# musaru/Fall_Multimodal

Hardware: AMD Instinct MI355X
Metric: clips/sec (fwd+bwd) 3-stream Fall3, B=256, 1/2/4/8 GPUs; top-1 acc parity (higher is better)
Workload: dtype bf16x3; 1 GPU; fall3_3stream_coco_mmpose_V18_S6_B256_per_gpu; global_batch=256, seq_len=30, parallelism=dp1, joints=18, imu_axes=6, classes=11, hip_graph=False, ranks=1

## Files before the change

fall_multimodal_amd/_lib.py:

```python
from __future__ import annotations

import ctypes
import os

import torch

HERE = os.path.dirname(os.path.abspath(__file__))
LIB_PATH = os.environ.get("F3_LIB") or os.path.join(HERE, "libfall3.so")

EXPORTS = (
    "f3_net_create", "f3_net_destroy", "f3_net_num_entries", "f3_net_entry", "f3_net_param_count",
    "f3_net_buffer_count", "f3_net_counter_count", "f3_net_workspace_bytes", "f3_net_forward",
    "f3_net_loss", "f3_net_backward", "f3_rmsprop_step", "f3_conv_forward", "f3_status_string",
    "f3_net_debug_tensor", "f3_conv_backward_data", "f3_conv_backward_weight", "f3_conv_wgrad_packed", "f3_split_x3cat",
    "f3_conv_forward_x3cat", "f3_conv_backward_data_x3cat", "f3_conv_backward_weight_x3cat", "f3_conv_step_x3cat", "f3_graph_mix_forward",
    "f3_graph_mix_backward", "f3_graph_mix_forward_ex", "f3_graph_mix_backward_ex", "f3_net_backward_phase",
    "f3_net_grad_split", "f3_net_wait_phase1", "f3_net_backward_rmsprop", "f3_net_fused_rmsprop", "f3_net_precision", "f3_net_status",
    "f3_targcn_create", "f3_targcn_destroy", "f3_targcn_num_entries", "f3_targcn_entry", "f3_targcn_param_count",
    "f3_targcn_buffer_count", "f3_targcn_workspace_bytes", "f3_targcn_forward", "f3_targcn_backward", "f3_targcn_stage_times", "f3_targcn_status", "f3_net_sensor_times", "f3_soft_ce",
    "f3_sktr_create", "f3_sktr_destroy", "f3_sktr_num_entries", "f3_sktr_entry", "f3_sktr_param_count",
    "f3_sktr_buffer_count", "f3_sktr_counter_count", "f3_sktr_workspace_bytes", "f3_sktr_forward", "f3_sktr_backward",
    "f3_musa_create", "f3_musa_destroy", "f3_musa_num_entries", "f3_musa_entry", "f3_musa_param_count",
    "f3_musa_buffer_count", "f3_musa_counter_count", "f3_musa_workspace_bytes", "f3_musa_forward", "f3_musa_backward",
    "f3_musa_guards",
    "f3_dwconv_t_forward", "f3_pointwise_conv", "f3_rgb_scratch_floats", "f3_rgb_forward", "f3_rgb_backward",
)

F3_OK, F3_EINVAL, F3_EBATCH, F3_EHIP, F3_ESTATE, F3_EDEVICE = 0, 1001, 1002, 1003, 1004, 1005
ENTRY_PARAM, ENTRY_BUFFER, ENTRY_COUNTER = 0, 1, 2


class F3TargcnConfig(ctypes.Structure):
    _fields_ = [(n, ctypes.c_int) for n in ("num_node", "num_class", "precision")]


class F3MusaConfig(ctypes.Structure):
    _fields_ = [(n, ctypes.c_int) for n in ("num_point", "frames", "num_class", "precision")]


class F3SktrConfig(ctypes.Structure):
    _fields_ = [(n, ctypes.c_int) for n in ("num_joint", "frames", "persons", "num_class", "precision")]


class F3Config(ctypes.Structure):
    _fields_ = [(n, ctypes.c_int) for n in (
        "model", "num_node", "num_partition", "num_class", "in_channels", "sensor", "sensor_dim",
        "sensor_classes", "softmax_output", "naming", "frames", "sensor_frames", "precision")]


# ... 14 lines not shown
        "f3_net_num_entries": (I, [P]),
        "f3_net_entry": (I, [P, I, ctypes.POINTER(ctypes.c_char_p), ctypes.POINTER(I), ctypes.POINTER(I),
                             ctypes.POINTER(I64), ctypes.POINTER(I64)]),
        "f3_net_param_count": (I64, [P]),
        "f3_net_buffer_count": (I64, [P]),
        "f3_net_counter_count": (I64, [P]),
        "f3_net_workspace_bytes": (I64, [P, I]),
        "f3_net_forward": (I, [P, I, I, P, P, P, P, P, P, P, P]),
        "f3_net_loss": (I, [P, I, P, P, P, P, P]),
        "f3_net_backward": (I, [P, I, P, P, P, P, P]),
        "f3_net_backward_phase": (I, [P, I, P, P, P, P, I, P]),
        "f3_net_grad_split": (I64, [P]),
        "f3_net_wait_phase1": (I, [P, P]),
        "f3_net_backward_rmsprop": (I, [P, I, P, P, P, P, P, F, F, F, P]),
        "f3_net_fused_rmsprop": (I, [P]),
        "f3_net_precision": (I, [P]),
        "f3_net_status": (I, [P, I]),
        "f3_rmsprop_step": (I, [P, P, P, I64, F, F, F, F, P]),
        "f3_conv_forward": (I, [P, P, P, P, P, I, I, I, I, I, I, I, I, I, P]),
        "f3_status_string": (ctypes.c_char_p, [I]),
        "f3_net_debug_tensor": (P, [P, I, P, I, I, ctypes.c_char_p]),
        "f3_conv_backward_data": (I, [P, P, P, P, I, I, I, I, I, I, I, I, I, P]),
        "f3_conv_backward_weight": (I, [P, P, P, P, I, I, I, I, I, I, I, I, I, P]),
        "f3_conv_wgrad_packed": (I, [P, P, P, ctypes.c_longlong, I, I, I, I, I, I, I, I, P]),
        "f3_split_x3cat": (I, [P, P, ctypes.c_int64, I, P]),
        "f3_conv_forward_x3cat": (I, [P, P, P, P, P, I, I, I, I, I, I, I, I, P]),
        "f3_conv_backward_data_x3cat": (I, [P, P, P, P, I, I, I, I, I, I, I, I, P]),
        "f3_conv_backward_weight_x3cat": (I, [P, P, P, P, I, I, I, I, I, I, I, I, P]),
        "f3_conv_step_x3cat": (I, [I, P, P, P, P, P, P, P, P, P, P, F, P, P, I, I, I, I, I, P]),
        "f3_graph_mix_forward": (I, [P, P, P, I, I, I, I, P]),
        "f3_graph_mix_backward": (I, [P, P, P, P, P, I, I, I, I, P]),
        "f3_graph_mix_forward_ex": (I, [P, P, P, I, I, I, I, I, P]),
        "f3_graph_mix_backward_ex": (I, [P, P, P, P, P, I, I, I, I, I, P]),
        "f3_targcn_create": (I, [ctypes.POINTER(F3TargcnConfig), ctypes.POINTER(P)]),
        "f3_targcn_destroy": (None, [P]),
        "f3_targcn_num_entries": (I, [P]),
        "f3_targcn_entry": (I, [P, I, ctypes.POINTER(ctypes.c_char_p), ctypes.POINTER(I), ctypes.POINTER(I),
                                ctypes.POINTER(I64), ctypes.POINTER(I64)]),
        "f3_targcn_param_count": (I64, [P]),
        "f3_targcn_buffer_count": (I64, [P]),
        "f3_targcn_workspace_bytes": (I64, [P, I]),
        "f3_targcn_stage_times": (I, [P, I, P]),
        "f3_targcn_status": (I, [P, I]),
        "f3_net_sensor_times": (I, [P, I, P]),
        "f3_targcn_forward": (I, [P, I, P, P, P, P, P, P]),
        "f3_targcn_backward": (I, [P, I, P, P, P, P, P, P]),
        "f3_soft_ce": (I, [P, P, I, I, P, P, P]),
        "f3_sktr_create": (I, [ctypes.POINTER(F3SktrConfig), ctypes.POINTER(P)]),
        "f3_sktr_destroy": (None, [P]),
        "f3_sktr_num_entries": (I, [P]),
        "f3_sktr_entry": (I, [P, I, ctypes.POINTER(ctypes.c_char_p), ctypes.POINTER(I), ctypes.POINTER(I),
                              ctypes.POINTER(I64), ctypes.POINTER(I64)]),
        "f3_sktr_param_count": (I64, [P]),
        "f3_sktr_buffer_count": (I64, [P]),
        "f3_sktr_counter_count": (I64, [P]),
        "f3_sktr_workspace_bytes": (I64, [P, I]),
        "f3_sktr_forward": (I, [P, I, I, P, P, P, P, P, P, P, ctypes.c_uint, F, P]),
        "f3_sktr_backward": (I, [P, I, P, P, P, P, P, P]),
        "f3_musa_create": (I, [ctypes.POINTER(F3MusaConfig), ctypes.POINTER(P)]),
        "f3_musa_destroy": (None, [P]),
        "f3_musa_num_entries": (I, [P]),
        "f3_musa_entry": (I, [P, I, ctypes.POINTER(ctypes.c_char_p), ctypes.POINTER(I), ctypes.POINTER(I),
                              ctypes.POINTER(I64), ctypes.POINTER(I64)]),
        "f3_musa_param_count": (I64, [P]),
        "f3_musa_buffer_count": (I64, [P]),
        "f3_musa_counter_count": (I64, [P]),
# ... 39 lines not shown
```

fall_multimodal_amd/csrc/layers.h:

```cpp
#pragma once
#include "common.h"

namespace f3 {

enum : int { PREP_MUL = 0, PREP_PACK_CONV, PREP_PACK_CONV_T, PREP_PACK_GCN, PREP_PACK_GCN_T, PREP_GCN_BIAS, PREP_COPY,
              PREP_UNPACK_CONV };

struct PrepJob {
  int type, n;
  float* dst;
  const float* s0;
  const float* s1;
  const float* s2;
  int d0, d1, d2;
  int bf16;
};

struct DataBnArgs {
  int N, T, V, C, motion;
  const float* skel;
  float* out;
  int act16;
  BnRef bn;
  double* st_sum;
  double* st_sq;
  const float* dout;
  float* dgamma;
  float* dbeta;
  float* part;
};

struct MixArgs {
  int K, V, Cin, frames;
  const float* A;
  const float* x;
  int x16;
  float* z;
  float* dx;
  float* dA;
  int accumulate;
  float* part;
  unsigned short* zb;
  const unsigned short* dzb;
  int no_colsum;
  int x3;
  unsigned short* z3;
};
constexpr int kMixParts = 1024;

struct Gcn0Args {
  int frames, K, V, Ci;
  const float* A;
  const unsigned short* x;
  const unsigned short* w;
  const float* beff;
  unsigned short* z;
  unsigned short* g;
  double* st_sum;
  double* st_sq;
  const unsigned short* dg;
  float* dx;
  int accumulate;
  float* part_dA;
  float* part_dW;
  int f32;
};

struct GcnBiasBwdArgs {
  int K, V, C;
  const float* Aeff;
  const float* A;
  const float* G;
  const float* bias;
  float* db;
  const float* dAeff;
  float* dE;
};

enum : int { RES_NONE = 0, RES_ID = 1, RES_CONV = 2 };

constexpr int kCaMaxRowsPerThread = 4;
// ... 97 lines not shown
  int bchunks;
};


struct BnRunJob {
  const double* sum;
  const double* sumsq;
  double count;
  int C;
  float* rmean;
  float* rvar;
  long long* nbt;
};

constexpr int kMaxPrepJobs = 56;
struct PrepTable {
  int n;
  PrepJob jobs[kMaxPrepJobs];
};
constexpr int kMaxBnJobs = 56;
struct BnRunTable {
  int n;
  BnRunJob jobs[kMaxBnJobs];
};

}

int f3_prep(const f3::PrepTable& t, hipStream_t s);
int f3_databn_fwd(const f3::DataBnArgs* a, hipStream_t s);
int f3_databn_bwd(const f3::DataBnArgs* a, hipStream_t s);
int f3_mix_fwd(const f3::MixArgs* a, hipStream_t s);
int f3_mix_bwd(const f3::MixArgs* a, hipStream_t s);
int f3_mix_bwd_parts(const f3::MixArgs* a);
bool f3_mix_lds_ok(int K, int V, int Cin);
bool f3_mix_x3_ok(int K, int V, int Cin);
int f3_split_x3(const float* x, unsigned short* out, long long rows, int C, hipStream_t s);
int f3_gcn_bias_bwd(const f3::GcnBiasBwdArgs* a, hipStream_t s);
bool f3_gcn0_ok(int K, int V, int Ci, int C);
int f3_gcn0_fwd(const f3::Gcn0Args* a, hipStream_t s);
int f3_gcn0_bwd(const f3::Gcn0Args* a, hipStream_t s);
int f3_gcn0_bwd_parts(const f3::Gcn0Args* a);
int f3_databn_bwd2(const f3::DataBnArgs* a, hipStream_t s);
int f3_block_out(f3::BlockArgs a, hipStream_t s);
int f3_block_bwd_reduce(f3::BlockArgs a, hipStream_t s);
int f3_block_bwd_apply(f3::BlockArgs a, hipStream_t s);
int f3_bn_bwd_apply(f3::BnBwdArgs a, hipStream_t s);
int f3_bn_bwd_parts(int N, int TV, int V);
int f3_block_chunks(int TV);
int f3_bnrelu_bf16(const f3::BnReluArgs* a, hipStream_t s);
constexpr int kColsumJobs = 10;
struct ColsumJob {
  const float* part;
  float* out;
  long long ld;
  int rows, cols;
};
int f3_colsum_multi(const ColsumJob* jobs, int n, hipStream_t s);
int f3_colsum(const float* part, int rows, int cols, float* out, hipStream_t s);
int f3_colsum_ld(const float* part, int rows, long long ld, int cols, float* out, hipStream_t s);
int f3_ca_fwd(const f3::CaArgs* a, hipStream_t s);
int f3_ca_bwd(const f3::CaArgs* a, hipStream_t s);
int f3_ca_bwd_weights(const f3::CaArgs* a, hipStream_t s, ColsumJob* defer = nullptr, int* ndefer = nullptr);
bool f3_ca_x_ok(int N, int C, int TV);
int f3_bn_running(const f3::BnRunTable& t, hipStream_t s);
```

fall_multimodal_amd/csrc/net.cpp:

```cpp
#include <hip/hip_runtime.h>

#include <algorithm>
#include <cstdio>
#include <functional>
#include <cstdlib>
#include <cstring>
#include <string>
#include <vector>

#include "common.h"
#include "status_ring.h"
#include "kernels.h"
#include "layers.h"
#include "sensor.h"
#include "fall3.h"

using namespace f3;

namespace {

struct Entry {
  std::string name;
  int kind;
  std::vector<int64_t> shape;
// ... 447 lines not shown
    r.gamma = p(bi.w);
    r.beta = p(bi.b);
    r.rmean = B ? b(bi.rm) : nullptr;
    r.rvar = B ? b(bi.rv) : nullptr;
    r.count = count;
    r.eval = eval;
    return r;
  }
};


ConvGeom geom(int M, int Nc, int Kc, int KT, int S, int P, int tr, int T_out, int T_in, int V, int lda, int ldo) {
  ConvGeom g;
  g.M = M; g.Nc = Nc; g.Kc = Kc; g.KT = KT; g.S = S; g.P = P; g.transposed = tr;
  g.T_out = T_out; g.T_in = T_in; g.V = V; g.lda = lda; g.ldo = ldo;
  return g;
}

void add_job(PrepTable& t, int type, int n, float* dst, const float* s0, const float* s1, const float* s2, int d0,
             int d1, int d2, int bf16 = 0) {
  PrepJob& j = t.jobs[t.n++];
  j.type = type; j.n = n; j.dst = dst; j.s0 = s0; j.s1 = s1; j.s2 = s2; j.d0 = d0; j.d1 = d1; j.d2 = d2;
  j.bf16 = bf16;
}

inline const unsigned short* bf(const float* p, int on) { return on ? reinterpret_cast<const unsigned short*>(p) : nullptr; }
inline int is_x3(const f3_net& n) { return n.cfg.precision == F3_PRECISION_BF16X3; }
inline int side_pct(bool split, int l) { return split && l >= 2 ? 75 : 0; }
constexpr int x3code() { return 4; }
inline int x3mul(int code) { return code == 4 ? 2 : 1; }
inline void x3_gemm(ConvGemmArgs& a, int C) {
  a.x3n = 1;
  a.g.lda = 2 * C;
}

inline int wcode(const f3_net& n) { return n.cfg.precision == F3_PRECISION_BF16 ? 1 : is_x3(n) ? 2 : 0; }
inline unsigned short* bfa(float* p, int on) { return on ? reinterpret_cast<unsigned short*>(p) : nullptr; }

void add_bnrun(BnRunTable& t, const Ptrs& q, const BnIdx& bi, const double* sum, const double* sq, double count) {
  BnRunJob& j = t.jobs[t.n++];
  j.sum = sum; j.sumsq = sq; j.count = count; j.C = bi.C;
  j.rmean = q.b(bi.rm); j.rvar = q.b(bi.rv); j.nbt = q.c(bi.nbt);
}

int stream_forward_layer(const f3_net& net, int si, int N, int train, const Ptrs& q, Ws& w, BnRunTable& run,
                         hipStream_t s, int l);

int stream_forward(const f3_net& net, int si, int N, int train, const Ptrs& q, Ws& w, const float* skel,
                   BnRunTable& run, hipStream_t s, int stage) {
  if (stage >= 0) return stream_forward_layer(net, si, N, train, q, w, run, s, stage);
  const StreamIdx& S = net.st[si];
  StreamWs& W = w.st[si];
  const int K = net.K, V = net.V, eval = !train;
  const int hb = net.cfg.precision == F3_PRECISION_BF16;
  const int wc = wcode(net);
  PrepTable pt;
  pt.n = 0;
  add_job(pt, PREP_COPY, K * V * V, W.A, q.b(S.A), nullptr, nullptr, 0, 0, 0);
  for (int l = 0; l < 7; ++l) {
    const LayerIdx& L = S.L[l];
    LayerWs& X = W.L[l];
    const int C = L.cout, Ci = L.cin;
    add_job(pt, PREP_MUL, K * V * V, X.aeff, q.b(S.A), q.p(L.edge), nullptr, 0, 0, 0);
    add_job(pt, PREP_GCN_BIAS, V * C, X.beff, q.b(S.A), q.p(L.edge), q.p(L.gcn_b), C, V, K);
    const bool l0f = wc == 2 && f3_gcn0_ok(K, V, Ci, C);
    const int xc = wc == 2 ? x3code() : wc;
// ... 220 lines not shown
    bb.dgamma = q.g(L.bn1.w); bb.dbeta = q.g(L.bn1.b); bb.dv = W.dv; bb.g = X.g; bb.dg = dg; bb.G = X.G;
    bb.Gpart = X.gpart; bb.dgb = bfa(dg, hb); bb.act16 = hb; bb.no_colsum = split;
    const bool gcat = x3 && f3_mix_x3_ok(K, V, Ci);
    if (gcat) { bb.dgb = bfa(dg, 1); bb.x3 = 1; }
    if (part & 1) F3_TRY(f3_bn_bwd_apply(bb, s));
    const bool g0 = (hb || x3) && f3_gcn0_ok(K, V, Ci, C);
    Gcn0Args b0;
    std::memset(&b0, 0, sizeof(b0));
    int g0_parts = 0;
    if (g0) {
      b0.frames = N * Ti; b0.K = K; b0.V = V; b0.Ci = Ci; b0.A = X.aeff;
      b0.x = reinterpret_cast<const unsigned short*>(X.x); b0.w = bf(X.gw, 1); b0.z = bfa(X.z, 1);
      b0.dg = bfa(dg, 1); b0.dx = dx; b0.accumulate = L.res == RES_ID;
      b0.f32 = x3;
      g0_parts = f3_gcn0_bwd_parts(&b0);
      if ((size_t)g0_parts * (K * V * V + K * C * Ci) > (size_t)kMixParts * K * V * V) return F3_EINVAL;
      b0.part_dA = X.mixpart;
      b0.part_dW = X.mixpart + (size_t)g0_parts * K * V * V;
    }
    ConvGemmArgs gd;
    std::memset(&gd, 0, sizeof(gd));
    gd.g = geom(Mi, K * Ci, C, 1, 1, 0, 0, Ti, Ti, V, C, K * Ci);
    gd.in = hb ? nullptr : dg; gd.inb = bfa(dg, hb); gd.zero = w.zero;
    gd.w = X.gwT; gd.wb = bf(X.gwT, wq); gd.x3 = x3; gd.out = W.dZ;
    if (gcat) {
      gd.x3 = 0; gd.in = nullptr; gd.inb = bfa(dg, 1);
      x3_gemm(gd, C);
    }
    const bool dzb = hb && f3_mix_lds_ok(K, V, Ci);
    if (dzb) {
      if (!f3_igemm_ok(gd)) return F3_EINVAL;
      gd.outb = bfa(W.dZ, 1);
    }
    if ((part & 1) && !g0) F3_TRY(f3_conv_gemm(&gd, 0, 0, s));
    MixArgs mx;
    std::memset(&mx, 0, sizeof(mx));
    mx.K = K; mx.V = V; mx.Cin = Ci; mx.frames = N * Ti; mx.A = X.aeff; mx.x = X.x; mx.z = W.dZ;
    mx.dx = dx; mx.dA = X.dAeff; mx.accumulate = L.res == RES_ID; mx.part = X.mixpart; mx.x16 = hb;
    mx.no_colsum = split; mx.x3 = x3;
    mx.dzb = dzb ? bfa(W.dZ, 1) : nullptr;
    if (part & 1) F3_TRY(g0 ? f3_gcn0_bwd(&b0, s) : f3_mix_bwd(&mx, s));
    if (L.res == RES_CONV) {
      ConvGemmArgs rd;
      std::memset(&rd, 0, sizeof(rd));
      rd.g = geom(Mi, Ci, C, 1, L.stride, 0, 1, Ti, To, V, C, Ci);
      rd.in = hb ? nullptr : dres; rd.inb = bfa(dres, hb); rd.zero = w.zero;
      rd.w = X.rwT; rd.wb = bf(X.rwT, wq); rd.x3 = x3; rd.out = dx;
      if (x3) {
        rd.x3 = 0; rd.in = nullptr; rd.inb = bfa(dres, 1);
        x3_gemm(rd, C);
      }
      if (part & 1) F3_TRY(f3_conv_gemm(&rd, 0, EPI_ADD, s));
    }
    if (split && (part & 1) && hipEventRecord(net.ev_main[si][l], s) != hipSuccess) return F3_EHIP;
    if (split && (part & 2) && hipStreamWaitEvent(ss, net.ev_main[si][l], 0) != hipSuccess) return F3_EHIP;
    WgradArgs tw;
    std::memset(&tw, 0, sizeof(tw));
    tw.wg_pct = side_pct(split, l);
    tw.g = geom(Mo, C, C, 9, L.stride, 4, 0, To, Ti, V, C, C);
    tw.ldy = C; tw.dw = q.g(L.tcn_w); tw.db = q.g(L.tcn_b);
    tw.outmap = WG_OUT_CONV; tw.bf16 = hb; tw.x3 = x3;
    if (hb) {
      tw.dyb = bfa(dh, 1); tw.inb = X.u; tw.zero = w.zero;
      tw.slab = W.slab; tw.slab_cap = kWgradSlabFloats; tw.dw_ref = q.g(L.tcn_w);
      if (!f3_wgrad_glds_ok(tw)) return F3_EINVAL;
      if (part & 2) F3_TRY(f3_conv_wgrad(&tw, 0, ss));
    } else if (x3) {
      tw.x3 = 0; tw.bf16 = 1;
      tw.ldy = 2 * C; tw.dyb = bfa(dh, 1); tw.inb = X.u; tw.zero = w.zero;
      tw.slab = W.slab; tw.slab_cap = kWgradSlabFloats * 4; tw.dw_ref = q.g(L.tcn_w);
      tw.g = geom(Mo, C, C, 9, L.stride, 4, 0, To, Ti, V, 2 * C, C);
      tw.x3seg = 1;
      tw.db = nullptr;
      if (!f3_wgrad_glds_ok(tw)) return F3_EINVAL;
// ... 4 lines not shown
        if (L.res == RES_CONV) cj[ncj++] = {X.dbpart + C, q.g(L.res_b), 2LL * C, rows, C};
      }
    } else {
      tw.dy = dh; tw.in = X.g; tw.pro_bn = bn1;
      if (part & 2) F3_TRY(f3_conv_wgrad(&tw, 1, ss));
    }
    ca.wpart = W.dets;
    if (part & 2) F3_TRY(f3_ca_bwd_weights(&ca, ss, cj, &ncj));
    if (L.res == RES_CONV) {
      WgradArgs rw;
      std::memset(&rw, 0, sizeof(rw));
      rw.wg_pct = side_pct(split, l);
      rw.g = geom(Mo, C, Ci, 1, L.stride, 0, 0, To, Ti, V, Ci, C);
      rw.ldy = C; rw.dw = q.g(L.res_w); rw.db = q.g(L.res_b); rw.outmap = WG_OUT_CONV; rw.bf16 = hb; rw.x3 = x3;
      if (hb) {
        rw.dyb = bfa(dres, 1); rw.inb = X.xb; rw.zero = w.zero;
        rw.slab = W.slab; rw.slab_cap = kWgradSlabFloats; rw.dw_ref = q.g(L.res_w);
      } else if (x3) {
        rw.x3 = 0; rw.bf16 = 1;
        rw.ldy = 2 * C; rw.dyb = bfa(dres, 1); rw.inb = X.xb; rw.zero = w.zero;
        rw.slab = W.slab; rw.slab_cap = kWgradSlabFloats * 4; rw.dw_ref = q.g(L.res_w);
        rw.g = geom(Mo, C, Ci, 1, L.stride, 0, 0, To, Ti, V, 2 * Ci, C);
        rw.x3seg = 1;
        rw.db = nullptr;
        if (!f3_wgrad_glds_ok(rw)) return F3_EINVAL;
      } else {
        rw.dy = dres; rw.in = X.x;
      }
      if (part & 2) F3_TRY(f3_conv_wgrad(&rw, 0, ss));
    }
    if (split) {
      const int T = L.T_in, fch = f3_bn_bwd_parts(N, T * V, V);
      if (part & 2) cj[ncj++] = {X.gpart, X.G, (long long)V * C, fch, V * C};
      const int mparts = g0 ? 0 : f3_mix_bwd_parts(&mx);
      if (mparts && (part & 2)) cj[ncj++] = {X.mixpart, X.dAeff, (long long)K * V * V, mparts, K * V * V};
    }
    if (g0 && (part & 2)) {
      cj[ncj++] = {b0.part_dA, X.dAeff, (long long)K * V * V, g0_parts, K * V * V};
      cj[ncj++] = {b0.part_dW, q.g(L.gcn_w), (long long)K * C * Ci, g0_parts, K * C * Ci};
    }
    if (ncj > kColsumJobs) return F3_EINVAL;
    F3_TRY(f3_colsum_multi(cj, ncj, ss));
    ncj = 0;
    WgradArgs gw;
    std::memset(&gw, 0, sizeof(gw));
    gw.wg_pct = side_pct(split, l);
    gw.g = geom(Mi, C, K * Ci, 1, 1, 0, 0, Ti, Ti, V, K * Ci, C);
    gw.ldy = C; gw.dw = q.g(L.gcn_w); gw.db = nullptr;
    if (hb) {
      gw.dyb = bfa(dg, 1); gw.inb = bfa(X.z, 1); gw.zero = w.zero;
    } else {
      gw.dy = dg; gw.in = X.z;
    }
    gw.outmap = WG_OUT_GCN; gw.gcn_cin = Ci; gw.bf16 = hb; gw.x3 = x3;
    if (gcat) {
      gw.x3 = 0; gw.bf16 = 1; gw.outmap = WG_OUT_CONV;
      gw.ldy = 2 * C; gw.dyb = bfa(dg, 1); gw.inb = bfa(X.z, 1); gw.zero = w.zero; gw.dy = nullptr; gw.in = nullptr;
      gw.slab = W.slab; gw.slab_cap = kWgradSlabFloats * 4; gw.dw_ref = q.g(L.gcn_w); gw.dw = nullptr;
      gw.g = geom(Mi, C, K * Ci, 1, 1, 0, 0, Ti, Ti, V, 2 * K * Ci, C);
      gw.x3seg = 1;
      if (!f3_wgrad_glds_ok(gw)) return F3_EINVAL;
    }
    if ((part & 2) && !g0) F3_TRY(f3_conv_wgrad(&gw, 0, ss));
    GcnBiasBwdArgs gb;
    gb.K = K; gb.V = V; gb.C = C; gb.Aeff = X.aeff; gb.A = W.A; gb.G = X.G; gb.bias = q.p(L.gcn_b);
    gb.db = q.g(L.gcn_b); gb.dAeff = X.dAeff; gb.dE = q.g(L.edge);
    if (part & 2) F3_TRY(f3_gcn_bias_bwd(&gb, ss));
// ... 853 lines not shown
  if ((flags & F3_MIX_Z3) && !(flags & F3_MIX_X3)) return F3_EINVAL;
  MixArgs m;
  std::memset(&m, 0, sizeof(m));
  m.K = K; m.V = V; m.Cin = Cin; m.frames = frames; m.A = A_eff;
  m.x = static_cast<const float*>(x); m.x16 = flags & F3_MIX_X_BF16; m.x3 = (flags & F3_MIX_X3) != 0;
  m.z = static_cast<float*>(z);
  if (flags & F3_MIX_Z_BF16) m.zb = static_cast<unsigned short*>(z);
  if (flags & F3_MIX_Z3) m.z3 = static_cast<unsigned short*>(z);
  return f3_mix_fwd(&m, (hipStream_t)stream);
}

int f3_graph_mix_backward_ex(const float* A_eff, const void* x, const void* dz, float* dx, float* dA, int frames, int K,
                             int V, int Cin, int flags, void* stream) {
  if (!A_eff || !x || !dz || !dx || !dA || frames < 0 || (flags & ~5) || ((flags & F3_MIX_X3) && (flags & 1)))
    return F3_EINVAL;
  hipStream_t s = (hipStream_t)stream;
  if (hipMemsetAsync(dA, 0, sizeof(float) * K * V * V, s) != hipSuccess) return F3_EHIP;
  MixArgs m;
  std::memset(&m, 0, sizeof(m));
  m.K = K; m.V = V; m.Cin = Cin; m.frames = frames; m.A = A_eff; m.x = static_cast<const float*>(x);
  m.dx = dx; m.dA = dA; m.accumulate = 0; m.x3 = (flags & F3_MIX_X3) != 0;
  if (flags & F3_MIX_X_BF16) {
    m.x16 = 1;
    m.dzb = static_cast<const unsigned short*>(dz);
  } else {
    m.z = const_cast<float*>(static_cast<const float*>(dz));
  }
  static float* part = nullptr;
  if (!part && hipMalloc(&part, sizeof(float) * kMixParts * 1024) != hipSuccess) return F3_EHIP;
  m.part = part;
  return f3_mix_bwd(&m, s);
}

void* f3_net_debug_tensor(f3_net* net, int batch, void* workspace, int stream, int layer, const char* what) {
  if (!net || stream < 0 || stream >= net->nstreams || layer < 0 || layer > 6) return nullptr;
  Ws w = plan(*net, batch, (char*)workspace);
  StreamWs& W = w.st[stream];
  LayerWs& X = W.L[layer];
  const std::string k(what);
  if (k == "x") return (void*)X.x;
  if (k == "z") return X.z;
  if (k == "g") return X.g;
  if (k == "h") return X.h;
  if (k == "r") return X.r;
  if (k == "out") return X.out;
  if (k == "att") return X.att;
  if (k == "dh") return X.dh;
  if (k == "u") return X.u;
  if (k == "dv") return W.dv;
  if (k == "dg") return X.dg;
  if (k == "dZ") return W.dZ;
  if (k == "dres") return X.dres;
  if (k == "dx0") return W.dx[0];
  if (k == "dx1") return W.dx[1];
  if (k == "bn1_fsum") return X.bn1.fsum;
  if (k == "bn1_fsq") return X.bn1.fsq;
  if (k == "bn1_bsum") return X.bn1.bsum;
  if (k == "bn1_bsq") return X.bn1.bsq;
  if (k == "twT") return X.twT;
  if (k == "P1") return X.P1;
  if (k == "P2") return X.P2;
  if (k == "e") return X.e;
  if (k == "gap") return X.gap;
  if (k == "q1") return X.q1;
  if (k == "hid") return X.hid;
  if (k == "dq1") return X.dq1;
// ... 27 lines not shown
```

include/fall3.h:

```cpp
#ifndef FALL3_H
#define FALL3_H
#include <stdint.h>

#ifdef __cplusplus
extern "C" {
#endif

#define F3_OK 0
#define F3_EINVAL 1001
#define F3_EBATCH 1002
#define F3_EHIP 1003
#define F3_ESTATE 1004
#define F3_EDEVICE 1005

enum { F3_MODEL_TWO_STGCAN_BILSTM = 0, F3_MODEL_TWO_STGCAN = 1, F3_MODEL_STGCN = 2, F3_MODEL_BILSTM = 3 };
enum { F3_SENSOR_NONE = 0, F3_SENSOR_BILSTM = 1, F3_SENSOR_CNN_BILSTM = 2 };
enum { F3_NAMING_PACKAGE = 0, F3_NAMING_NOTEBOOK = 1 };
enum { F3_PRECISION_FP32 = 0,
       F3_PRECISION_BF16 = 1,
       F3_PRECISION_BF16_FP32IN = 2,
       F3_PRECISION_BF16X3 = 4  };
enum { F3_ENTRY_PARAM = 0, F3_ENTRY_BUFFER = 1, F3_ENTRY_COUNTER = 2 };

typedef struct f3_config {
// ... 65 lines not shown

#define F3_STEP_GCN_FWD 0
#define F3_STEP_TCN_DGRAD 1
int f3_split_x3cat(const float* x, void* out, int64_t rows, int C, void* stream);
int f3_conv_forward_x3cat(const void* x3, const float* w, const float* bias, float* out, void* wpack, int N, int T_in,
                          int V, int Cin, int Cout, int KT, int stride, int pad, void* stream);
int f3_conv_backward_data_x3cat(const void* dy3, const float* w, float* dx, void* wpack, int N, int T_in, int V,
                                int Cin, int Cout, int KT, int stride, int pad, void* stream);
int f3_conv_backward_weight_x3cat(const void* dy3, const void* x3, float* dw, float* db, int N, int T_in, int V,
                                  int Cin, int Cout, int KT, int stride, int pad, void* stream);
int f3_conv_step_x3cat(int kind, const void* in3, const float* w, void* wpack, float* out, const float* bias_v,
                       const float* g, const float* gamma, const float* beta, const double* bn_sum,
                       const double* bn_sq, float bn_count, double* st_sum, double* st_sq, int N, int T, int V,
                       int Cin, int Cout, void* stream);

int f3_pointwise_conv(const void* x, const void* wpack, const float* bias, void* out, int out_bf16, double* st_sum,
                      double* st_sq, int N, int T_in, int T_out, int V, int Cin, int Cout, int stride, int transposed,
                      int epi, void* stream);

long long f3_rgb_scratch_floats(int B, int T);
int f3_rgb_forward(const void* frames, const void* wpack, const float* bias, float* feat, int B, int T, void* stream);
int f3_rgb_backward(const void* frames, const void* wpack, const float* bias, const float* dfeat, float* dw, float* db,
                    float* scratch, long long scratch_floats, int B, int T, void* stream);

int f3_graph_mix_forward(const float* A_eff, const float* x, float* z, int frames, int K, int V, int Cin,
                         void* stream);
int f3_graph_mix_backward(const float* A_eff, const float* x, const float* dz, float* dx, float* dA, int frames, int K,
                          int V, int Cin, void* stream);
enum { F3_MIX_X_BF16 = 1, F3_MIX_Z_BF16 = 2, F3_MIX_X3 = 4, F3_MIX_Z3 = 8 };
int f3_graph_mix_forward_ex(const float* A_eff, const void* x, void* z, int frames, int K, int V, int Cin, int flags,
                            void* stream);
int f3_graph_mix_backward_ex(const float* A_eff, const void* x, const void* dz, float* dx, float* dA, int frames, int K,
                             int V, int Cin, int flags, void* stream);

const char* f3_status_string(int status);

typedef struct f3_targcn_config {
  int num_node;
  int num_class;
  int precision;
} f3_targcn_config;

typedef struct f3_targcn f3_targcn;

int f3_targcn_create(const f3_targcn_config* cfg, f3_targcn** out);
void f3_targcn_destroy(f3_targcn* net);
int f3_targcn_num_entries(const f3_targcn* net);
int f3_targcn_entry(const f3_targcn* net, int i, const char** name, int* kind, int* ndim, int64_t* shape8,
                    int64_t* offset);
int64_t f3_targcn_param_count(const f3_targcn* net);
int64_t f3_targcn_buffer_count(const f3_targcn* net);
int64_t f3_targcn_workspace_bytes(const f3_targcn* net, int batch);
int f3_targcn_forward(f3_targcn* net, int batch, const float* params, const float* buffers, const float* source,
                      float* out, void* workspace, void* stream);
int f3_targcn_backward(f3_targcn* net, int batch, const float* params, const float* buffers, const float* dout,
                       float* grads, void* workspace, void* stream);
int f3_targcn_stage_times(f3_targcn* net, int enable, float* ms);
int f3_targcn_status(f3_targcn* net, int wait);
int f3_soft_ce(const float* out, const float* label, int N, int C, float* loss, float* dout, void* stream);

typedef struct f3_musa_config {
  int num_point;
  int frames;
  int num_class;
  int precision;
} f3_musa_config;
// ... 52 lines not shown
```

Before: 31940 clips/s.

## Fuse GCN data-gradient GEMM with graph-mix backward in one x3 kernel

Adds a persistent HIP kernel that computes the GCN weight data-gradient (dZ = W^T·dg) with bf16x3 MFMA and feeds it straight through LDS into the graph-mix backward, producing dx and per-workgroup dA partials in one pass. It replaces the separate conv GEMM plus mix-backward launches when Cin is 64 and the x3 concat path is active. This removes the dZ round trip through global memory and one launch per layer. In exchange it relies on a complex LDS layout and transposed reads, and it is gated by an environment flag that defaults to on.

```diff
diff --git a/fall_multimodal_amd/_lib.py b/fall_multimodal_amd/_lib.py
--- a/fall_multimodal_amd/_lib.py
+++ b/fall_multimodal_amd/_lib.py
@@ -14,7 +14,8 @@
     "f3_net_loss", "f3_net_backward", "f3_rmsprop_step", "f3_conv_forward", "f3_status_string",
     "f3_net_debug_tensor", "f3_conv_backward_data", "f3_conv_backward_weight", "f3_conv_wgrad_packed", "f3_split_x3cat",
     "f3_conv_forward_x3cat", "f3_conv_backward_data_x3cat", "f3_conv_backward_weight_x3cat", "f3_conv_step_x3cat", "f3_graph_mix_forward",
-    "f3_graph_mix_backward", "f3_graph_mix_forward_ex", "f3_graph_mix_backward_ex", "f3_net_backward_phase",
+    "f3_graph_mix_backward", "f3_graph_mix_forward_ex", "f3_graph_mix_backward_ex", "f3_gcn_dgrad_mix_x3",
+    "f3_net_backward_phase",
     "f3_net_grad_split", "f3_net_wait_phase1", "f3_net_backward_rmsprop", "f3_net_fused_rmsprop", "f3_net_precision", "f3_net_status",
     "f3_targcn_create", "f3_targcn_destroy", "f3_targcn_num_entries", "f3_targcn_entry", "f3_targcn_param_count",
     "f3_targcn_buffer_count", "f3_targcn_workspace_bytes", "f3_targcn_forward", "f3_targcn_backward", "f3_targcn_stage_times", "f3_targcn_status", "f3_net_sensor_times", "f3_soft_ce",
@@ -95,6 +96,7 @@
         "f3_graph_mix_backward": (I, [P, P, P, P, P, I, I, I, I, P]),
         "f3_graph_mix_forward_ex": (I, [P, P, P, I, I, I, I, I, P]),
         "f3_graph_mix_backward_ex": (I, [P, P, P, P, P, I, I, I, I, I, P]),
+        "f3_gcn_dgrad_mix_x3": (I, [P, P, P, P, P, P, P, I, I, I, I, I, I, I, P]),
         "f3_targcn_create": (I, [ctypes.POINTER(F3TargcnConfig), ctypes.POINTER(P)]),
         "f3_targcn_destroy": (None, [P]),
         "f3_targcn_num_entries": (I, [P]),
diff --git a/fall_multimodal_amd/csrc/gcn_bwd.hip b/fall_multimodal_amd/csrc/gcn_bwd.hip
--- /dev/null
+++ b/fall_multimodal_amd/csrc/gcn_bwd.hip
@@ -0,0 +1,345 @@
+#include "igemm.h"
+#include "layers.h"
+
+#include <algorithm>
+#include <cstring>
+
+namespace f3 {
+
+typedef __bf16 gb_bf16x4 __attribute__((ext_vector_type(4)));
+typedef short gb_s16x4 __attribute__((ext_vector_type(4)));
+typedef __attribute__((address_space(3))) const char gb_lds_t;
+
+F3_DEV void gb_a_split(float t, __bf16& hi, __bf16& lo) {
+  const float h = __uint_as_float(__float_as_uint(t) & 0xffff0000u);
+  hi = __builtin_bit_cast(__bf16, (unsigned short)(__float_as_uint(h) >> 16));
+  lo = (__bf16)(t - h);
+}
+
+F3_DEV void gb_split4_store(const f32x4 v, char* hi, char* lo) {
+  gb_bf16x4 h, l;
+#pragma unroll
+  for (int e = 0; e < 4; ++e) {
+    h[e] = (__bf16)v[e];
+    l[e] = (__bf16)(v[e] - (float)h[e]);
+  }
+  *reinterpret_cast<gb_bf16x4*>(hi) = h;
+  *reinterpret_cast<gb_bf16x4*>(lo) = l;
+}
+
+F3_DEV f32x4 gb_mfma_x3(bf16x8 ah, bf16x8 al, bf16x8 bh, bf16x8 bl, f32x4 c) {
+  c = mfma_bf16x(al, bh, c);
+  c = mfma_bf16x(ah, bl, c);
+  return mfma_bf16x(ah, bh, c);
+}
+
+F3_DEV f32x4 gb_mfma_dz(bf16x8 wh, bf16x8 wl, bf16x8 gh, bf16x8 gl, f32x4 c) {
+  c = mfma_bf16x(wh, gh, c);
+  c = mfma_bf16x(wh, gl, c);
+  return mfma_bf16x(wl, gh, c);
+}
+
+F3_DEV void gb_barrier() {
+  asm volatile("s_waitcnt lgkmcnt(0)" ::: "memory");
+  __builtin_amdgcn_s_barrier();
+}
+
+constexpr int kGbRB = 144, kGbXR = 32, kGbZR = 64, kGbKmax = 3, kGbDxLd = 68;
+constexpr int gb_groups(int C) { return C == 256 ? 2 : 1; }
+constexpr int gb_threads(int C) { return 256 * gb_groups(C); }
+
+template <int C, bool ACC>
+__global__ __launch_bounds__(gb_threads(C)) __attribute__((amdgpu_waves_per_eu(C == 64 ? 3 : 1)))
+void gcn_dgrad_mix_x3_kernel(GcnDgradMixArgs a) {
+  constexpr int RB = kGbRB, GB = 4 * C + 16, G16 = C / 4;
+  constexpr int NG = gb_groups(C), NT = gb_threads(C);
+  constexpr bool ALDS = C == 64;
+  constexpr int KSL = C / 32 / NG;
+  constexpr int MTL = 2 / NG;
+  constexpr int PX = 512 / NT, PG = 8 * C / NT;
+  extern __shared__ __attribute__((aligned(16))) char smb[];
+  char* xh = smb;
+  char* xl = xh + kGbXR * RB;
+  char* zh = xl + kGbXR * RB;
+  char* zl = zh + kGbZR * RB;
+  char* gs = zl + kGbZR * RB;
+  float* dxs = reinterpret_cast<float*>(gs);
+  f32x4* red = reinterpret_cast<f32x4*>(gs + kGbXR * GB);
+  const int lane = threadIdx.x & 63, wave = threadIdx.x >> 6, tid = threadIdx.x;
+  const int wq = wave & 3, g = NG == 2 ? wave >> 2 : 0;
+  const int fr = lane & 15, fg = lane >> 4;
+  const int K = a.K, V = a.V, KV = K * V, Cin = a.Cin;
+  const int nch = Cin >> 6;
+  const int lin = xcd_remap(blockIdx.x, gridDim.x);
+  const int slot = lin / nch, j = lin - slot * nch, slots = gridDim.x / nch;
+  const int nx = V * 16, ng = V * G16;
+  const bool two = V > 16;
+
+  bf16x8 wh[kGbKmax][KSL], wl[kGbKmax][KSL];
+#pragma unroll
+  for (int k = 0; k < kGbKmax; ++k)
+#pragma unroll
+    for (int ks = 0; ks < KSL; ++ks) {
+      const __bf16* row =
+          reinterpret_cast<const __bf16*>(a.w) + ((size_t)min(k, K - 1) * Cin + 64 * j + 16 * wq + fr) * 2 * C;
+      wh[k][ks] = *reinterpret_cast<const bf16x8*>(row + 64 * (g * KSL + ks) + 8 * fg);
+      wl[k][ks] = *reinterpret_cast<const bf16x8*>(row + 64 * (g * KSL + ks) + 32 + 8 * fg);
+    }
+  {
+    float* At = reinterpret_cast<float*>(zh);
+    for (int e = tid; e < KV * V; e += NT) At[e] = a.A[e];
+    gb_barrier();
+  }
+  bf16x8 ahi[MTL][2], alo[MTL][2];
+#pragma unroll
+  for (int ml = 0; ml < MTL; ++ml)
+#pragma unroll
+    for (int ks = 0; ks < 2; ++ks)
+#pragma unroll
+      for (int e = 0; e < 8; ++e) {
+        __bf16 h, l;
+        const int wk = 32 * ks + 8 * fg + e, v = 16 * (NG == 2 ? g : ml) + fr;
+        const int w = wk / K, k = wk - w * K;
+        const bool in = wk < KV && v < V;
+        const float t = reinterpret_cast<const float*>(zh)[in ? (k * V + v) * V + w : 0];
+        gb_a_split(in ? t : 0.f, h, l);
+        ahi[ml][ks][e] = h;
+        alo[ml][ks][e] = l;
+      }
+  bf16x8* afr = reinterpret_cast<bf16x8*>(gs + kGbXR * GB);
+  if constexpr (ALDS) {
+    if (wave == 0) {
+#pragma unroll
+      for (int ml = 0; ml < MTL; ++ml)
+#pragma unroll
+        for (int ks = 0; ks < 2; ++ks) {
+          afr[(ml * 2 + ks) * 64 + lane] = ahi[ml][ks];
+          afr[(MTL * 2 + ml * 2 + ks) * 64 + lane] = alo[ml][ks];
+        }
+    }
+  }
+  gb_barrier();
+  for (int o = KV * RB + tid * 16; o < kGbZR * RB; o += NT * 16) {
+    *reinterpret_cast<f32x4*>(zh + o) = f32x4{0.f, 0.f, 0.f, 0.f};
+    *reinterpret_cast<f32x4*>(zl + o) = f32x4{0.f, 0.f, 0.f, 0.f};
+  }
+  for (int o = V * RB + tid * 16; o < kGbXR * RB; o += NT * 16) {
+    *reinterpret_cast<f32x4*>(xh + o) = f32x4{0.f, 0.f, 0.f, 0.f};
+    *reinterpret_cast<f32x4*>(xl + o) = f32x4{0.f, 0.f, 0.f, 0.f};
+  }
+  for (int o = V * GB + tid * 16; o < kGbXR * GB; o += NT * 16)
+    *reinterpret_cast<f32x4*>(gs + o) = f32x4{0.f, 0.f, 0.f, 0.f};
+  f32x4 dacc[MTL];
+#pragma unroll
+  for (int ml = 0; ml < MTL; ++ml) dacc[ml] = f32x4{0.f, 0.f, 0.f, 0.f};
+  f32x4 rx[PX], rg[PG], ro[PX];
+  auto prefetch = [&](int f) {
+    const float* xg = a.x + (size_t)f * V * Cin + 64 * j;
+    const f32x4* gg = reinterpret_cast<const f32x4*>(reinterpret_cast<const __bf16*>(a.dg) + (size_t)f * V * 2 * C);
+#pragma unroll
+    for (int q = 0; q < PX; ++q) {
+      const int i = min(tid + q * NT, nx - 1);
+      rx[q] = *reinterpret_cast<const f32x4*>(xg + (size_t)(i >> 4) * Cin + (i & 15) * 4);
+    }
+#pragma unroll
+    for (int q = 0; q < PG; ++q) rg[q] = gg[min(tid + q * NT, ng - 1)];
+  };
+  prefetch(slot);
+  for (int f = slot; f < a.frames; f += slots) {
+    gb_barrier();
+#pragma unroll
+    for (int q = 0; q < PX; ++q) {
+      const int i = tid + q * NT;
+      if (i < nx) {
+        const int o = (i >> 4) * RB + (i & 15) * 8;
+        gb_split4_store(rx[q], xh + o, xl + o);
+      }
+    }
+#pragma unroll
+    for (int q = 0; q < PG; ++q) {
+      const int i = tid + q * NT;
+      if (i < ng) *reinterpret_cast<f32x4*>(gs + (i / G16) * GB + (i % G16) * 16) = rg[q];
+    }
+    gb_barrier();
+    float* dxf = a.dx + (size_t)f * V * Cin + 64 * j;
+    if (ACC) {
+#pragma unroll
+      for (int q = 0; q < PX; ++q) {
+        const int i = min(tid + q * NT, nx - 1);
+        ro[q] = *reinterpret_cast<const f32x4*>(dxf + (size_t)(i >> 4) * Cin + (i & 15) * 4);
+      }
+    }
+    prefetch(min(f + slots, a.frames - 1));
+    f32x4 acc[2][kGbKmax];
+#pragma unroll
+    for (int mt = 0; mt < 2; ++mt)
+#pragma unroll
+      for (int k = 0; k < kGbKmax; ++k) acc[mt][k] = f32x4{0.f, 0.f, 0.f, 0.f};
+#pragma unroll
+    for (int mt = 0; mt < 2; ++mt) {
+      if (mt == 0 || two) {
+#pragma unroll
+        for (int ks = 0; ks < KSL; ++ks) {
+          const char* p = gs + (16 * mt + fr) * GB + (32 * (g * KSL + ks) + 8 * fg) * 2;
+          const bf16x8 gh = *reinterpret_cast<const bf16x8*>(p);
+          const bf16x8 gl = *reinterpret_cast<const bf16x8*>(p + 2 * C);
+#pragma unroll
+          for (int k = 0; k < kGbKmax; ++k)
+            if (k < K) acc[mt][k] = gb_mfma_dz(wh[k][ks], wl[k][ks], gh, gl, acc[mt][k]);
+        }
+      }
+    }
+    f32x4 fin[MTL][kGbKmax];
+    if constexpr (NG == 2) {
+#pragma unroll
+      for (int k = 0; k < kGbKmax; ++k) red[(wave * kGbKmax + k) * 64 + lane] = g ? acc[0][k] : acc[1][k];
+      gb_barrier();
+#pragma unroll
+      for (int k = 0; k < kGbKmax; ++k)
+        fin[0][k] = (g ? acc[1][k] : acc[0][k]) + red[((wave ^ 4) * kGbKmax + k) * 64 + lane];
+    } else {
+#pragma unroll
+      for (int ml = 0; ml < MTL; ++ml)
+#pragma unroll
+        for (int k = 0; k < kGbKmax; ++k) fin[ml][k] = acc[ml][k];
+    }
+#pragma unroll
+    for (int ml = 0; ml < MTL; ++ml)
+#pragma unroll
+      for (int k = 0; k < kGbKmax; ++k) {
+        const int w = 16 * (NG == 2 ? g : ml) + fr;
+        if (k < K && w < V) {
+          const int o = (w * K + k) * RB + (16 * wq + 4 * fg) * 2;
+          gb_split4_store(fin[ml][k], zh + o, zl + o);
+        }
+      }
+    gb_barrier();
+    {
+      bf16x8 bh[2], bl[2];
+#pragma unroll
+      for (int ks = 0; ks < 2; ++ks) {
+        const int o = (32 * ks + 8 * fg + (fr >> 2)) * RB + 32 * wq + 8 * (fr & 3);
+        const unsigned ph = (unsigned)(size_t)(gb_lds_t*)(zh + o), pl = (unsigned)(size_t)(gb_lds_t*)(zl + o);
+        gb_s16x4 h0, h1, l0, l1;
+        asm volatile("ds_read_b64_tr_b16 %0, %1" : "=v"(h0) : "v"(ph));
+        asm volatile("ds_read_b64_tr_b16 %0, %1 offset:%2" : "=v"(h1) : "v"(ph), "n"(4 * RB));
+        asm volatile("ds_read_b64_tr_b16 %0, %1" : "=v"(l0) : "v"(pl));
+        asm volatile("ds_read_b64_tr_b16 %0, %1 offset:%2" : "=v"(l1) : "v"(pl), "n"(4 * RB));
+        asm volatile("s_waitcnt lgkmcnt(0)" : "+v"(h0), "+v"(h1), "+v"(l0), "+v"(l1)::"memory");
+        bh[ks] = __builtin_bit_cast(bf16x8, __builtin_shufflevector(h0, h1, 0, 1, 2, 3, 4, 5, 6, 7));
+        bl[ks] = __builtin_bit_cast(bf16x8, __builtin_shufflevector(l0, l1, 0, 1, 2, 3, 4, 5, 6, 7));
+      }
+#pragma unroll
+      for (int ml = 0; ml < MTL; ++ml) {
+        f32x4 xa = f32x4{0.f, 0.f, 0.f, 0.f};
+#pragma unroll
+        for (int ks = 0; ks < 2; ++ks) {
+          const bf16x8 ah = ALDS ? afr[(ml * 2 + ks) * 64 + lane] : ahi[ml][ks];
+          const bf16x8 al = ALDS ? afr[(MTL * 2 + ml * 2 + ks) * 64 + lane] : alo[ml][ks];
+          xa = gb_mfma_x3(ah, al, bh[ks], bl[ks], xa);
+        }
+        const int mt = NG == 2 ? g : ml;
+#pragma unroll
+        for (int r = 0; r < 4; ++r) dxs[(16 * mt + 4 * fg + r) * kGbDxLd + 16 * wq + fr] = xa[r];
+      }
+    }
+#pragma unroll
+    for (int ks = 0; ks < 2; ++ks) {
+      const int cb = (32 * ks + 8 * fg) * 2;
+      const bf16x8 z_h = *reinterpret_cast<const bf16x8*>(zh + (16 * wq + fr) * RB + cb);
+      const bf16x8 z_l = *reinterpret_cast<const bf16x8*>(zl + (16 * wq + fr) * RB + cb);
+#pragma unroll
+      for (int ml = 0; ml < MTL; ++ml) {
+        const int mt = NG == 2 ? g : ml;
+        const bf16x8 x_h = *reinterpret_cast<const bf16x8*>(xh + (16 * mt + fr) * RB + cb);
+        const bf16x8 x_l = *reinterpret_cast<const bf16x8*>(xl + (16 * mt + fr) * RB + cb);
+        dacc[ml] = gb_mfma_x3(x_h, x_l, z_h, z_l, dacc[ml]);
+      }
+    }
+    gb_barrier();
+#pragma unroll
+    for (int q = 0; q < PX; ++q) {
+      const int i = min(tid + q * NT, nx - 1);
+      f32x4 v = *reinterpret_cast<const f32x4*>(dxs + (i >> 4) * kGbDxLd + (i & 15) * 4);
+      if (ACC) v += ro[q];
+      *reinterpret_cast<f32x4*>(dxf + (size_t)(i >> 4) * Cin + (i & 15) * 4) = v;
+    }
+  }
+  float* row = a.part + (size_t)lin * K * V * V;
+#pragma unroll
+  for (int ml = 0; ml < MTL; ++ml)
+#pragma unroll
+    for (int r = 0; r < 4; ++r) {
+      const int v = 16 * (NG == 2 ? g : ml) + 4 * fg + r, wk = 16 * wq + fr;
+      if (v < V && wk < KV) {
+        const int w = wk / K, k = wk - w * K;
+        row[(k * V + v) * V + w] = dacc[ml][r];
+      }
+    }
+}
+
+template <int C>
+static size_t gb_lds() {
+  return (size_t)2 * (kGbXR + kGbZR) * kGbRB + (size_t)kGbXR * (4 * C + 16) +
+         (gb_groups(C) == 2 ? (size_t)8 * kGbKmax * 64 * 16 : 0) + (C == 64 ? (size_t)8 * 64 * 16 : 0);
+}
+
+template <int C>
+static int gb_slots() {
+  static const int slots = [] {
+    int per_cu[2] = {0, 0}, dev = 0, cus = 256;
+    const void* fn[2] = {(const void*)gcn_dgrad_mix_x3_kernel<C, false>, (const void*)gcn_dgrad_mix_x3_kernel<C, true>};
+    for (int i = 0; i < 2; ++i) {
+      (void)hipFuncSetAttribute(fn[i], hipFuncAttributeMaxDynamicSharedMemorySize, (int)gb_lds<C>());
+      if (hipOccupancyMaxActiveBlocksPerMultiprocessor(&per_cu[i], fn[i], gb_threads(C), gb_lds<C>()) != hipSuccess ||
+          per_cu[i] < 1)
+        per_cu[i] = 1;
+    }
+    if (hipGetDevice(&dev) == hipSuccess) (void)hipDeviceGetAttribute(&cus, hipDeviceAttributeMultiprocessorCount, dev);
+    (void)hipGetLastError();
+    return std::min(per_cu[0], per_cu[1]) * cus;
+  }();
+  return slots;
+}
+
+static int gb_grid(const GcnDgradMixArgs* a) {
+  const int nch = a->Cin / 64;
+  int wgs = a->C == 64 ? gb_slots<64>() : a->C == 128 ? gb_slots<128>() : gb_slots<256>();
+  wgs = std::min(a->max_workgroups > 0 ? a->max_workgroups : wgs, kMixParts);
+  const int slots = std::max(1, std::min(a->frames, wgs / nch));
+  return slots * nch;
+}
+
+template <int C>
+static int gb_launch(const GcnDgradMixArgs* a, int grid, hipStream_t s) {
+  if (a->accumulate)
+    hipLaunchKernelGGL((gcn_dgrad_mix_x3_kernel<C, true>), dim3(grid), dim3(gb_threads(C)), gb_lds<C>(), s, *a);
+  else
+    hipLaunchKernelGGL((gcn_dgrad_mix_x3_kernel<C, false>), dim3(grid), dim3(gb_threads(C)), gb_lds<C>(), s, *a);
+  F3_LAUNCH_CHECK();
+  return F3_OK;
+}
+
+}
+
+using namespace f3;
+
+bool f3_gcn_dgrad_mix_ok(int K, int V, int Cin, int C) {
+  const auto ch = [](int c) { return c == 64 || c == 128 || c == 256; };
+  return K >= 1 && K <= kGbKmax && V >= 1 && V <= 32 && K * V <= 64 && ch(Cin) && ch(C) && C >= Cin;
+}
+
+int f3_gcn_dgrad_mix_parts(const GcnDgradMixArgs* a) {
+  if (!f3_gcn_dgrad_mix_ok(a->K, a->V, a->Cin, a->C) || a->frames <= 0) return 0;
+  return gb_grid(a);
+}
+
+int f3_gcn_dgrad_mix(const GcnDgradMixArgs* a, hipStream_t s) {
+  if (!f3_gcn_dgrad_mix_ok(a->K, a->V, a->Cin, a->C)) return F3_EINVAL;
+  if (!a->dg || !a->w || !a->A || !a->x || !a->dx || !a->part) return F3_EINVAL;
+  if (a->frames <= 0) return F3_OK;
+  const int grid = gb_grid(a);
+  F3_TRY(a->C == 64 ? gb_launch<64>(a, grid, s) : a->C == 128 ? gb_launch<128>(a, grid, s) : gb_launch<256>(a, grid, s));
+  if (a->no_colsum) return F3_OK;
+  return f3_colsum(a->part, grid, a->K * a->V * a->V, a->dA, s);
+}
diff --git a/fall_multimodal_amd/csrc/layers.h b/fall_multimodal_amd/csrc/layers.h
--- a/fall_multimodal_amd/csrc/layers.h
+++ b/fall_multimodal_amd/csrc/layers.h
@@ -47,6 +47,20 @@
   unsigned short* z3;
 };
 constexpr int kMixParts = 1024;
+
+struct GcnDgradMixArgs {
+  int frames, K, V, Cin, C;
+  const unsigned short* dg;
+  const unsigned short* w;
+  const float* A;
+  const float* x;
+  float* dx;
+  float* dA;
+  int accumulate;
+  float* part;
+  int no_colsum;
+  int max_workgroups;
+};
 
 struct Gcn0Args {
   int frames, K, V, Ci;
@@ -210,6 +224,9 @@
 int f3_mix_fwd(const f3::MixArgs* a, hipStream_t s);
 int f3_mix_bwd(const f3::MixArgs* a, hipStream_t s);
 int f3_mix_bwd_parts(const f3::MixArgs* a);
+bool f3_gcn_dgrad_mix_ok(int K, int V, int Cin, int C);
+int f3_gcn_dgrad_mix(const f3::GcnDgradMixArgs* a, hipStream_t s);
+int f3_gcn_dgrad_mix_parts(const f3::GcnDgradMixArgs* a);
 bool f3_mix_lds_ok(int K, int V, int Cin);
 bool f3_mix_x3_ok(int K, int V, int Cin);
 int f3_split_x3(const float* x, unsigned short* out, long long rows, int C, hipStream_t s);
diff --git a/fall_multimodal_amd/csrc/net.cpp b/fall_multimodal_amd/csrc/net.cpp
--- a/fall_multimodal_amd/csrc/net.cpp
+++ b/fall_multimodal_amd/csrc/net.cpp
@@ -503,6 +503,11 @@
 inline void x3_gemm(ConvGemmArgs& a, int C) {
   a.x3n = 1;
   a.g.lda = 2 * C;
+}
+
+inline bool gcn_dgrad_fused() {
+  static const bool on = !getenv("F3_GCN_DGRAD_FUSED") || atoi(getenv("F3_GCN_DGRAD_FUSED")) != 0;
+  return on;
 }
 
 inline int wcode(const f3_net& n) { return n.cfg.precision == F3_PRECISION_BF16 ? 1 : is_x3(n) ? 2 : 0; }
@@ -789,14 +794,23 @@
       if (!f3_igemm_ok(gd)) return F3_EINVAL;
       gd.outb = bfa(W.dZ, 1);
     }
-    if ((part & 1) && !g0) F3_TRY(f3_conv_gemm(&gd, 0, 0, s));
+    const bool gfuse = gcat && !g0 && Ci == 64 && gcn_dgrad_fused() && f3_gcn_dgrad_mix_ok(K, V, Ci, C);
+    GcnDgradMixArgs gf;
+    std::memset(&gf, 0, sizeof(gf));
+    if (gfuse) {
+      gf.frames = N * Ti; gf.K = K; gf.V = V; gf.Cin = Ci; gf.C = C; gf.dg = bfa(dg, 1); gf.w = bf(X.gwT, 1);
+      gf.A = X.aeff; gf.x = X.x; gf.dx = dx; gf.dA = X.dAeff; gf.accumulate = L.res == RES_ID;
+      gf.part = X.mixpart; gf.no_colsum = split;
+    }
+    if ((part & 1) && !g0 && !gfuse) F3_TRY(f3_conv_gemm(&gd, 0, 0, s));
     MixArgs mx;
     std::memset(&mx, 0, sizeof(mx));
     mx.K = K; mx.V = V; mx.Cin = Ci; mx.frames = N * Ti; mx.A = X.aeff; mx.x = X.x; mx.z = W.dZ;
     mx.dx = dx; mx.dA = X.dAeff; mx.accumulate = L.res == RES_ID; mx.part = X.mixpart; mx.x16 = hb;
     mx.no_colsum = split; mx.x3 = x3;
     mx.dzb = dzb ? bfa(W.dZ, 1) : nullptr;
-    if (part & 1) F3_TRY(g0 ? f3_gcn0_bwd(&b0, s) : f3_mix_bwd(&mx, s));
+    if (gfuse) gf.max_workgroups = f3_mix_bwd_parts(&mx);
+    if (part & 1) F3_TRY(g0 ? f3_gcn0_bwd(&b0, s) : gfuse ? f3_gcn_dgrad_mix(&gf, s) : f3_mix_bwd(&mx, s));
     if (L.res == RES_CONV) {
       ConvGemmArgs rd;
       std::memset(&rd, 0, sizeof(rd));
@@ -867,7 +881,7 @@
     if (split) {
       const int T = L.T_in, fch = f3_bn_bwd_parts(N, T * V, V);
       if (part & 2) cj[ncj++] = {X.gpart, X.G, (long long)V * C, fch, V * C};
-      const int mparts = g0 ? 0 : f3_mix_bwd_parts(&mx);
+      const int mparts = g0 ? 0 : gfuse ? f3_gcn_dgrad_mix_parts(&gf) : f3_mix_bwd_parts(&mx);
       if (mparts && (part & 2)) cj[ncj++] = {X.mixpart, X.dAeff, (long long)K * V * V, mparts, K * V * V};
     }
     if (g0 && (part & 2)) {
@@ -1787,6 +1801,30 @@
   return f3_mix_bwd(&m, s);
 }
 
+int f3_gcn_dgrad_mix_x3(const void* dg3, const float* w, void* wpack, const float* A_eff, const float* x, float* dx,
+                        float* dA, int frames, int K, int V, int Cin, int C, int accumulate, int max_workgroups,
+                        void* stream) {
+  hipStream_t s = (hipStream_t)stream;
+  if (!dg3 || !wpack || !A_eff || !x || !dx || !dA || frames < 0 || max_workgroups < 0) return F3_EINVAL;
+  if (!f3_gcn_dgrad_mix_ok(K, V, Cin, C) || K * V * V > 1024) return F3_EINVAL;
+  if (w) {
+    PrepTable t;
+    t.n = 0;
+    add_job(t, PREP_PACK_CONV_T, C * K * Cin * x3mul(x3code()), static_cast<float*>(wpack), w, nullptr, nullptr, C,
+            K * Cin, 1, x3code());
+    F3_TRY(f3_prep(t, s));
+  }
+  if (hipMemsetAsync(dA, 0, sizeof(float) * K * V * V, s) != hipSuccess) return F3_EHIP;
+  static float* part = nullptr;
+  if (!part && hipMalloc(&part, sizeof(float) * kMixParts * 1024) != hipSuccess) return F3_EHIP;
+  GcnDgradMixArgs a;
+  std::memset(&a, 0, sizeof(a));
+  a.frames = frames; a.K = K; a.V = V; a.Cin = Cin; a.C = C; a.dg = static_cast<const unsigned short*>(dg3);
+  a.w = static_cast<const unsigned short*>(wpack); a.A = A_eff; a.x = x; a.dx = dx; a.dA = dA;
+  a.accumulate = accumulate != 0; a.part = part; a.max_workgroups = max_workgroups;
+  return f3_gcn_dgrad_mix(&a, s);
+}
+
 void* f3_net_debug_tensor(f3_net* net, int batch, void* workspace, int stream, int layer, const char* what) {
   if (!net || stream < 0 || stream >= net->nstreams || layer < 0 || layer > 6) return nullptr;
   Ws w = plan(*net, batch, (char*)workspace);
diff --git a/include/fall3.h b/include/fall3.h
--- a/include/fall3.h
+++ b/include/fall3.h
@@ -121,6 +121,9 @@
                             void* stream);
 int f3_graph_mix_backward_ex(const float* A_eff, const void* x, const void* dz, float* dx, float* dA, int frames, int K,
                              int V, int Cin, int flags, void* stream);
+int f3_gcn_dgrad_mix_x3(const void* dg3, const float* w, void* wpack, const float* A_eff, const float* x, float* dx,
+                        float* dA, int frames, int K, int V, int Cin, int C, int accumulate, int max_workgroups,
+                        void* stream);
 
 const char* f3_status_string(int status);
 
```

Result: faster. 32650 clips/s, median of 6 (+2.2%).
